# Anonymousijcai2024ttnet/scale_imagenet

Hardware: AMD Instinct MI355X
Metric: images/sec ImageNet 224x224, TT-small, MI355X; top-1 exact-match (higher is better)
Workload: dtype u16/u32/u64 packed bits (gate path); f32 as prescaled fp16x2 split operands on the 16-bit MFMA (stem, lin1, lin2); 1 GPU; TT_general_imagenet_v2_small forward, batch=256 224x224 per GPU, bit-packed HIP LUT kernels (BASELINE.json configs[1]); batch_per_gpu=256, global_batch=256, batches_in_flight=2, input=float32 NCHW, normalised (the reference's contract), parallelism=batch shard x1

## Files before the change

scale_imagenet_amd/csrc/head.hip:

```cpp

#include <algorithm>
#include <cmath>
#include <type_traits>

#include "ttnet_common.h"

namespace ttnet {

namespace {

typedef float f32x16 __attribute__((ext_vector_type(16)));

typedef _Float16 f16x8 __attribute__((ext_vector_type(8)));
constexpr int NP = SPLIT_PLANES;

#ifndef TT_LIN1_SKIP
#define TT_LIN1_SKIP 0
#endif
constexpr int kLin1Skip = TT_LIN1_SKIP;

#ifndef TT_LIN1_BM
#define TT_LIN1_BM 128
#endif
#ifndef TT_LIN1_WGS
#define TT_LIN1_WGS 256
#endif
constexpr int G_BM = TT_LIN1_BM, G_BN = 128;
constexpr int G_MT = G_BM / 32, G_NT = G_BN / 32;
constexpr int G_KS = 1;
constexpr int G_CHUNK = 1024;
constexpr int G_STAGE = (G_MT + G_NT) * G_KS * NP * G_CHUNK;
#ifndef TT_LIN1_STAGES
#define TT_LIN1_STAGES 4
#endif
constexpr int G_STAGES = TT_LIN1_STAGES;
#ifndef TT_LIN1_WAVES
#define TT_LIN1_WAVES (TT_LIN1_BM / 32)
#endif
constexpr int G_WAVES = TT_LIN1_WAVES;
constexpr int G_WN = G_WAVES / G_MT, NPW = G_NT / G_WN;
static_assert(G_WAVES % G_MT == 0 && G_NT % G_WN == 0, "waves tile the workgroup's output");
constexpr int G_CHUNKS = (G_MT + G_NT) * G_KS * NP;
#ifndef TT_LIN1_LOADERS
#define TT_LIN1_LOADERS 0
#endif
constexpr int G_LOADERS = TT_LIN1_LOADERS;
constexpr int G_THREADS = 64 * (G_WAVES + G_LOADERS);
constexpr int G_LW = G_LOADERS ? G_LOADERS : G_WAVES;
constexpr int G_LOADS = (G_CHUNKS + G_LW - 1) / G_LW;
constexpr int G_LDS = G_STAGES * G_STAGE + G_CHUNK;

#ifdef TT_LIN1_STAMP
__device__ unsigned long long g_lin1_stamps[512][2];
#endif
template <int AUX_A, int AUX_B>
__global__ __launch_bounds__(G_THREADS) void gemm_f16x2_kernel(const uint8_t *__restrict__ Af, const uint8_t *__restrict__ Bf,
                                                         float *__restrict__ part, int M, int N, int KS, int ks_per,
                                                         int n_tiles, int m_tiles, int splits) {
  extern __shared__ __align__(16) uint8_t lds[];
  const int lane = threadIdx.x & 63, wave = __builtin_amdgcn_readfirstlane(threadIdx.x >> 6);
  const bool loader = G_LOADERS ? wave >= G_WAVES : true, consumer = wave < G_WAVES;
  const int lw = G_LOADERS ? (loader ? wave - G_WAVES : 0) : wave;
  int ntile, mtile, slice;
  {
    const int b = blockIdx.x, groups = m_tiles * splits;
    const int lanes8 = groups < 8 ? groups : 8;
    const int round = b / (lanes8 * n_tiles), rem = b % (lanes8 * n_tiles);
    int grp = round * lanes8 + rem % lanes8;
    ntile = rem / lanes8;
    if (round == groups / lanes8) {
      const int left = groups - round * lanes8;
      grp = round * lanes8 + rem % left;
      ntile = rem / left;
    }
    mtile = grp / splits;
    slice = grp % splits;
  }
  const int mt0 = mtile * G_MT, nt0 = ntile * G_NT;
  const int ks_beg = slice * ks_per, iters = ks_per / G_KS;

  const uint8_t *chunk_src[G_LOADS];
  int chunk_lds[G_LOADS];
#pragma unroll
  for (int jj = 0; jj < G_LOADS; ++jj) {
    const int c = lw + G_LW * jj;
    const bool real = c < G_CHUNKS;
    const bool isA = c < G_MT * G_KS * NP;
    const int cc = real ? (isA ? c : c - G_MT * G_KS * NP) : 0;
    const int pl = cc % NP, kk = (cc / NP) % G_KS, tl = cc / (NP * G_KS);
    chunk_src[jj] = (isA || !real ? Af : Bf) +
                    ((((size_t)((isA || !real ? mt0 : nt0) + tl) * KS + ks_beg + kk) * NP + pl) * 64 + lane) * 16;
    chunk_lds[jj] = real ? c * G_CHUNK : -1;
  }
  auto issue = [&](int it, int buf) {
    static_for<0, G_LOADS>([&](auto jc) {
      constexpr int jj = decltype(jc)::value;
      constexpr bool allA = G_LW * jj + G_LW - 1 < G_MT * G_KS * NP, allB = G_LW * jj >= G_MT * G_KS * NP;
      if constexpr (kLin1Skip & 3) {
        const bool isA = lw + G_LW * jj < G_MT * G_KS * NP;
        if (((kLin1Skip & 1) && isA) || ((kLin1Skip & 2) && !isA)) return;
      }
      const auto src = (const __attribute__((address_space(1))) void *)(chunk_src[jj] + (size_t)it * (G_KS * NP * G_CHUNK));
      const auto dst = (__attribute__((address_space(3))) void *)(lds + (chunk_lds[jj] >= 0 ? buf * G_STAGE + chunk_lds[jj] : G_STAGES * G_STAGE));
      if constexpr (allA) __builtin_amdgcn_global_load_lds(src, dst, 16, 0, AUX_A);
      else if constexpr (allB) __builtin_amdgcn_global_load_lds(src, dst, 16, 0, AUX_B);
      else __builtin_amdgcn_global_load_lds(src, dst, 16, 0, 0);
    });
  };

  constexpr int MPW = 1;
  const int wm = wave % G_MT, wn = wave / G_MT;
  f32x16 acc[MPW][NPW];
#pragma unroll
  for (int i = 0; i < MPW; ++i)
#pragma unroll
    for (int j = 0; j < NPW; ++j)
#pragma unroll
      for (int r = 0; r < 16; ++r) acc[i][j][r] = 0.f;

  static_assert(G_KS == 1 && MPW == 1 && NPW == 4, "the fragment pipeline below is written for one k-step per stage and four N-tiles per wave");
  auto wait_landed = [&](int younger) {
    if (younger >= 5) asm volatile("s_waitcnt vmcnt(%0)" ::"n"(5 * G_LOADS) : "memory");
    else if (younger == 4) asm volatile("s_waitcnt vmcnt(%0)" ::"n"(4 * G_LOADS) : "memory");
    else if (younger == 3) asm volatile("s_waitcnt vmcnt(%0)" ::"n"(3 * G_LOADS) : "memory");
    else if (younger == 2) asm volatile("s_waitcnt vmcnt(%0)" ::"n"(2 * G_LOADS) : "memory");
    else if (younger == 1) asm volatile("s_waitcnt vmcnt(%0)" ::"n"(G_LOADS) : "memory");
    else asm volatile("s_waitcnt vmcnt(0)" ::: "memory");
  };
  static_assert(G_STAGES >= 4 && G_STAGES <= 8 && 5 * G_LOADS < 64, "G_STAGES - 1 stages issued ahead; the barrier of k-step it frees slot (it - 1) % G_STAGES");
#ifdef TT_LIN1_STAMP
  const unsigned long long st_c = __builtin_amdgcn_s_memtime(), st_r = __builtin_amdgcn_s_memrealtime();
#endif
  if (loader) {
    for (int p = 0; p < G_STAGES - 1 && p < iters; ++p) issue(p, p);
    wait_landed(min(G_STAGES - 2, iters - 1));
  }
  __builtin_amdgcn_s_barrier();
  typedef uint32_t u32x4 __attribute__((ext_vector_type(4)));
  u32x4 af[2][NP], bq[NPW][NP];
#define TT_DSRD(dst, addr, off) asm volatile("ds_read_b128 %0, %1 offset:%2" : "=&v"(dst) : "v"(addr), "n"(off))
  const uint32_t lds0 = (uint32_t)(uintptr_t)(__attribute__((address_space(3))) void *)lds + (uint32_t)lane * 16u;
  const uint32_t offA = (uint32_t)(wm * NP) * G_CHUNK, offB = (uint32_t)(G_MT * NP + wn * NPW * NP) * G_CHUNK;
  auto tile = [&](int j, const u32x4 (&a_cur)[NP]) {
    if constexpr (kLin1Skip & 4) {
      acc[0][j][0] += __uint_as_float(a_cur[0][0] ^ bq[j][0][0] ^ bq[j][1][0] ^ a_cur[1][0]);
    } else {
      const f16x8 a0 = __builtin_bit_cast(f16x8, a_cur[0]), a1 = __builtin_bit_cast(f16x8, a_cur[1]);
      const f16x8 b0 = __builtin_bit_cast(f16x8, bq[j][0]), b1 = __builtin_bit_cast(f16x8, bq[j][1]);
      acc[0][j] = __builtin_amdgcn_mfma_f32_32x32x16_f16(a1, b0, acc[0][j], 0, 0, 0);
      acc[0][j] = __builtin_amdgcn_mfma_f32_32x32x16_f16(a0, b1, acc[0][j], 0, 0, 0);
      acc[0][j] = __builtin_amdgcn_mfma_f32_32x32x16_f16(a0, b0, acc[0][j], 0, 0, 0);
    }
    __builtin_amdgcn_sched_barrier(0);
  };
  auto kstep = [&](auto par_c, int it) {
    constexpr int P = decltype(par_c)::value;
    u32x4 (&a_cur)[NP] = af[P];
    u32x4 (&a_nxt)[NP] = af[1 - P];
    const uint32_t sb = lds0 + (uint32_t)(it % G_STAGES) * G_STAGE + offB;
    const uint32_t sn = lds0 + (uint32_t)((it + 1) % G_STAGES) * G_STAGE;
    const uint32_t snb = sn + offB, sna = sn + offA;
    TT_DSRD(bq[2][0], sb, 4 * G_CHUNK);
    TT_DSRD(bq[2][1], sb, 5 * G_CHUNK);
    asm volatile("s_waitcnt lgkmcnt(4)" : "+v"(bq[0][0]), "+v"(bq[0][1]), "+v"(a_cur[0]), "+v"(a_cur[1]));
    tile(0, a_cur);
    TT_DSRD(bq[3][0], sb, 6 * G_CHUNK);
    TT_DSRD(bq[3][1], sb, 7 * G_CHUNK);
    asm volatile("s_waitcnt lgkmcnt(4)" : "+v"(bq[1][0]), "+v"(bq[1][1]));
    tile(1, a_cur);
    TT_DSRD(bq[0][0], snb, 0);
    TT_DSRD(bq[0][1], snb, G_CHUNK);
    TT_DSRD(a_nxt[0], sna, 0);
    TT_DSRD(a_nxt[1], sna, G_CHUNK);
    asm volatile("s_waitcnt lgkmcnt(6)" : "+v"(bq[2][0]), "+v"(bq[2][1]));
    tile(2, a_cur);
    TT_DSRD(bq[1][0], snb, 2 * G_CHUNK);
    TT_DSRD(bq[1][1], snb, 3 * G_CHUNK);
    asm volatile("s_waitcnt lgkmcnt(6)" : "+v"(bq[3][0]), "+v"(bq[3][1]));
    tile(3, a_cur);
  };
  if (consumer) {
    const uint32_t s0 = lds0;
    TT_DSRD(bq[0][0], s0 + offB, 0);
    TT_DSRD(bq[0][1], s0 + offB, G_CHUNK);
    TT_DSRD(af[0][0], s0 + offA, 0);
    TT_DSRD(af[0][1], s0 + offA, G_CHUNK);
    TT_DSRD(bq[1][0], s0 + offB, 2 * G_CHUNK);
    TT_DSRD(bq[1][1], s0 + offB, 3 * G_CHUNK);
  }
  auto step = [&](auto par_c, int it) {
    if (loader) wait_landed(max(0, min(it + G_STAGES - 2, iters - 1) - (it + 1)));
    __builtin_amdgcn_s_barrier();
    if (loader && it + G_STAGES - 1 < iters) issue(it + G_STAGES - 1, (it + G_STAGES - 1) % G_STAGES);
    if (consumer) kstep(par_c, it);
  };
#pragma unroll 1
  for (int it = 0; it < iters; it += 2) {
    step(std::integral_constant<int, 0>{}, it);
    if (it + 1 < iters) step(std::integral_constant<int, 1>{}, it + 1);
  }
  if (consumer)
    asm volatile("s_waitcnt lgkmcnt(0)" : "+v"(bq[0][0]), "+v"(bq[0][1]), "+v"(bq[1][0]), "+v"(bq[1][1]), "+v"(af[0][0]), "+v"(af[0][1]),
                 "+v"(af[1][0]), "+v"(af[1][1]));
#undef TT_DSRD
#ifdef TT_LIN1_STAMP
  if (threadIdx.x == 0 && blockIdx.x < 512) {
    g_lin1_stamps[blockIdx.x][0] = __builtin_amdgcn_s_memtime() - st_c;
    g_lin1_stamps[blockIdx.x][1] = 10ull * (__builtin_amdgcn_s_memrealtime() - st_r);
  }
#endif
  if (!consumer) return;
  float4 *dst = (float4 *)part + (size_t)slice * (m_tiles * G_MT) * (n_tiles * G_NT) * 256;
#pragma unroll
  for (int i = 0; i < MPW; ++i)
#pragma unroll
    for (int j = 0; j < NPW; ++j) {
      float4 *tile = dst + ((size_t)(mt0 + wm + i) * (n_tiles * G_NT) + nt0 + wn * NPW + j) * 256 + lane;
#pragma unroll
      for (int g = 0; g < 4; ++g) {
        if ((kLin1Skip & 8) && g) continue;
        tile[g * 64] = make_float4(acc[i][j][4 * g], acc[i][j][4 * g + 1], acc[i][j][4 * g + 2], acc[i][j][4 * g + 3]);
      }
    }
}

__global__ void split_to_frag_kernel(const float *__restrict__ src, uint16_t *__restrict__ dst, int R, int K, int tiles,
                                     float prescale, int ld, int kvalid) {
  const size_t i = (size_t)blockIdx.x * blockDim.x + threadIdx.x;
  const int KS = K / 16;
  if (i >= (size_t)tiles * KS * 64 * 8) return;
  const int j = i % 8, ln = (i / 8) % 64;
  const size_t tk = i / 512;
  const int ks = tk % KS, tl = tk / KS;
  const int row = tl * 32 + (ln & 31), k = ks * 16 + 8 * (ln >> 5) + j;
  const float v = row < R && k < kvalid ? src[(size_t)row * ld + k] * prescale : 0.f;
  uint16_t h1, h2;
  split_f16x2(v, h1, h2);
  const size_t base = ((size_t)tl * KS + ks) * NP;
  dst[((base + 0) * 64 + ln) * 8 + j] = h1;
  dst[((base + 1) * 64 + ln) * 8 + j] = h2;
}

__global__ void frag_to_ref_kernel(const uint16_t *__restrict__ af, float *__restrict__ out, int n, int G, int PP) {
  const size_t t = (size_t)blockIdx.x * blockDim.x + threadIdx.x;
  const size_t per = (size_t)G * PP * 16;
  if (t >= (size_t)n * per) return;
  const int kk = t % 16, pp = (t / 16) % PP, g = (t / (16 * (size_t)PP)) % G;
  const int img = t / per;
  out[(size_t)img * per + ((size_t)(16 * g + kk)) * PP + pp] = load_feature(af, img, G * PP, g * PP + pp, kk);
}

__global__ void head_mid_kernel(const float4 *__restrict__ part, int splits, const float *__restrict__ scale,
                                const float *__restrict__ shift, uint16_t *__restrict__ mid_frag, int M, int N,
                                int polynomial, uint32_t *range_flag, int mt32, int nt32) {
  const size_t i = (size_t)blockIdx.x * blockDim.x + threadIdx.x;
  const size_t per_slice = (size_t)mt32 * nt32 * 256;
// ... 53 lines not shown
        const f16x8 b0 = __builtin_bit_cast(f16x8, fb[sl][0]), b1 = __builtin_bit_cast(f16x8, fb[sl][1]);
        acc = __builtin_amdgcn_mfma_f32_32x32x16_f16(a1, b0, acc, 0, 0, 0);
        acc = __builtin_amdgcn_mfma_f32_32x32x16_f16(a0, b1, acc, 0, 0, 0);
        acc = __builtin_amdgcn_mfma_f32_32x32x16_f16(a0, b0, acc, 0, 0, 0);
        if (i0 + sl + L2_STAGES < nk) load(i0 + sl + L2_STAGES, fa[sl], fb[sl]);
      }
    });
  }
#pragma unroll
  for (int r = 0; r < 16; ++r) red[(wave * 16 + r) * 64 + lane] = acc[r];
  __syncthreads();
  for (int e = threadIdx.x; e < 16 * 64; e += 64 * L2_WAVES) {
    double sum = 0.0;
#pragma unroll
    for (int w = 0; w < L2_WAVES; ++w) sum += (double)red[w * (16 * 64) + e];
    const int ln = e & 63, r = e >> 6;
    const int row = mt * 32 + (r & 3) + 8 * (r >> 2) + 4 * (ln >> 5);
    const int col = nt * 32 + (ln & 31);
    if (row < M && col < N) out[(size_t)row * N + col] = (float)(sum * (double)inv + (double)bias[col]);
  }
}

__global__ void permute_lin1_kernel(const float *__restrict__ w1, float *__restrict__ w1p, int O, int G, int PP) {
  const size_t i = (size_t)blockIdx.x * blockDim.x + threadIdx.x;
  const size_t K = (size_t)G * PP * 16;
  if (i >= (size_t)O * K) return;
  const size_t o = i / K, f = i % K;
  const int k = f % 16, pp = (f / 16) % PP, g = f / (16 * (size_t)PP);
  w1p[i] = w1[o * K + ((size_t)(16 * g + k)) * PP + pp];
}

}

int gemm_f16x2_splits(int M, int N, int KS) {
  const int tiles = ((M + G_BM - 1) / G_BM) * ((N + G_BN - 1) / G_BN);
  const int want = std::max(TT_LIN1_WGS / std::max(1, tiles), 8);
  for (int s = std::min(std::min(want, KS / 8), 128); s > 1; --s)
    if (KS % s == 0) return s;
  return 1;
}

size_t gemm_f16x2_part_elems(int M, int N, int KS) {
  const size_t mt = (M + G_BM - 1) / G_BM, nt = (N + G_BN - 1) / G_BN;
  return (size_t)gemm_f16x2_splits(M, N, KS) * mt * G_BM * nt * G_BN;
}

int launch_gemm_f16x2(const void *Af, const void *Bf, float *part, int M, int N, int K, int splits, hipStream_t s) {
  const int KS = K / 16;
  if (K % 16 || KS % splits || (KS / splits) % G_KS) {
    set_error("gemm_f16x2: K=%d not divisible into %d slices of %d k-steps", K, splits, G_KS);
    return TTNET_E_UNSUPPORTED;
  }
  static const int nt = getenv("TTNET_LIN1_NT") ? atoi(getenv("TTNET_LIN1_NT")) : 0;
  const int n_tiles = (N + G_BN - 1) / G_BN, m_tiles = (M + G_BM - 1) / G_BM;
  auto launch = [&](auto kernel) -> int {
    TT_TRY(ensure_dynamic_lds((const void *)kernel, G_LDS));
    hipLaunchKernelGGL(kernel, dim3(n_tiles * m_tiles * splits), dim3(G_THREADS), G_LDS, s, (const uint8_t *)Af, (const uint8_t *)Bf, part, M, N,
                       KS, KS / splits, n_tiles, m_tiles, splits);
    return TTNET_OK;
  };
  if (nt == 11) TT_TRY(launch(gemm_f16x2_kernel<2, 2>));
  else if (nt == 1) TT_TRY(launch(gemm_f16x2_kernel<0, 2>));
  else if (nt == 10) TT_TRY(launch(gemm_f16x2_kernel<2, 0>));
  else TT_TRY(launch(gemm_f16x2_kernel<0, 0>));
  TT_HIP(hipGetLastError());
  return TTNET_OK;
}

size_t frag_elems(int rows, int K) { return (size_t)((rows + 31) / 32) * (K / 16) * NP * 64 * 8; }

float weight_prescale(const float *w, size_t n) {
  float amax = 0.f;
  for (size_t i = 0; i < n; ++i) amax = fmaxf(amax, fabsf(w[i]));
  if (!(amax > 0.f) || !std::isfinite(amax)) return 1.0f;
  int e;
  frexpf(amax, &e);
  int k = 14 - e;
  k = k > 60 ? 60 : (k < -60 ? -60 : k);
  return ldexpf(1.0f, k);
}

int launch_split_to_frag(const float *src, void *dst, int R, int K, int rows_padded, float prescale, hipStream_t s, int ld,
                         int kvalid) {
  if (K % 16) {
    set_error("split_to_frag: K=%d is not a multiple of 16", K);
    return TTNET_E_UNSUPPORTED;
  }
  const int tiles = (rows_padded + 31) / 32;
  const size_t t = (size_t)tiles * (K / 16) * 64 * 8;
  hipLaunchKernelGGL(split_to_frag_kernel, dim3((unsigned)((t + 255) / 256)), dim3(256), 0, s, src, (uint16_t *)dst, R, K, tiles,
                     prescale, ld > 0 ? ld : K, kvalid > 0 ? kvalid : K);
  TT_HIP(hipGetLastError());
  return TTNET_OK;
}

int launch_frag_to_reference_order(const void *af, float *out, int n, int G, int PP, hipStream_t s) {
  const size_t t = (size_t)n * G * PP * 16;
  hipLaunchKernelGGL(frag_to_ref_kernel, dim3((unsigned)((t + 255) / 256)), dim3(256), 0, s, (const uint16_t *)af, out, n, G, PP);
  TT_HIP(hipGetLastError());
  return TTNET_OK;
}

int launch_head_mid(const float *part, int splits, const float *scale, const float *shift, void *mid_frag, int M, int N,
                    int polynomial, uint32_t *range_flag, hipStream_t s) {
  const int mt32 = (M + G_BM - 1) / G_BM * G_MT, nt32 = (N + G_BN - 1) / G_BN * G_NT;
  const size_t t = (size_t)mt32 * nt32 * 256;
  hipLaunchKernelGGL(head_mid_kernel, dim3((unsigned)((t + 255) / 256)), dim3(256), 0, s, (const float4 *)part, splits, scale, shift,
                     (uint16_t *)mid_frag, M, N, polynomial, range_flag, mt32, nt32);
  TT_HIP(hipGetLastError());
  return TTNET_OK;
}

int launch_lin2_f16x2(const void *mid_frag, const void *w2f, const float *bias, float inv, float *out, int M, int N, int K,
                      hipStream_t s) {
  const int KS = (K + 15) / 16;
  hipLaunchKernelGGL(lin2_f16x2_kernel, dim3((N + 31) / 32, (M + 31) / 32), dim3(64 * L2_WAVES), 0, s,
                     (const uint4 *)mid_frag, (const uint4 *)w2f, bias, inv, out, M, N, KS);
  TT_HIP(hipGetLastError());
  return TTNET_OK;
}

int launch_permute_lin1(const float *w1, float *w1p, int O, int G, int PP, hipStream_t s) {
  const size_t t = (size_t)O * G * PP * 16;
  hipLaunchKernelGGL(permute_lin1_kernel, dim3((unsigned)((t + 255) / 256)), dim3(256), 0, s, w1, w1p, O, G, PP);
  TT_HIP(hipGetLastError());
  return TTNET_OK;
}

}
```

scale_imagenet_amd/csrc/plan.hip:

```cpp

#include <dlfcn.h>
#include <math.h>
#include <stdarg.h>
#include <stdint.h>
#include <stdio.h>
#include <stdlib.h>
#include <string.h>

#include <algorithm>
#include <array>
#include <map>
#include <memory>

#include <mutex>
#include <unordered_map>

#include "ttnet_common.h"

namespace ttnet {

static thread_local char g_err[1024] = "";

void set_error(const char *fmt, ...) {
  va_list ap;
// ... 411 lines not shown
        for (int b = 0; b < 4; ++b) TT_TRY(dev_alloc(pl, &bw.o[b], 8, true, ws));
        if (mh.last) TT_TRY(dev_alloc(pl, &bw.idx, (size_t)nb * (mh.C / 8) * mh.Ho * mh.Wo, true, ws));
        continue;
      }
      TT_TRY(dev_alloc(pl, &L.x_rp[i], (size_t)nb * mh.C * mh.H, true, ws));
      TT_TRY(dev_alloc(pl, &L.x_cp[i], path == GatePath::Full ? 8 : (size_t)nb * mh.H * mh.W * (mh.C / 16), true, ws));
      if (path == GatePath::Full) TT_TRY(dev_alloc(pl, &bw.c3_tmp, (size_t)nb * mh.C * mh.H, true, ws));
      for (int b = 0; b < 4; ++b) {
        const size_t words16 = (size_t)nb * mh.Ho * mh.Wo * (mh.C / 16), rows64 = (size_t)nb * mh.C * mh.Ho;
        TT_TRY(dev_alloc(pl, &bw.o[b], (path == GatePath::XSmall || path == GatePath::Full) ? rows64 * 4 : words16, true, ws));
      }
    }
    if (path == GatePath::Full) {
      const MultiHead &lb = pl->blocks.back();
      TT_TRY(dev_alloc(pl, &L.last_float, (size_t)nb * lb.cf.g.out_planes * lb.Ho * lb.Wo, true, ws));
      size_t cap = 0;
      for (const MultiHead &mh : pl->blocks) {
        cap = std::max(cap, (size_t)mh.c3.g.groups * mh.H * mh.W);
        if (!mh.last) cap = std::max(cap, (size_t)mh.cf.g.groups * mh.Ho * mh.Wo);
      }
      pl->full_fix_cap = cap * (size_t)nb;
      TT_TRY(dev_alloc(pl, &L.full_fix, 64 + pl->full_fix_cap, true, ws));
      if (!pl->full_gel) {
        TT_TRY(dev_alloc(pl, &pl->full_gel, full_gelu_tables_elems(), false, ws));
        TT_TRY(launch_full_gelu_tables(pl->full_gel, nullptr));
        TT_HIP(hipDeviceSynchronize());
      }
    }
  }
  const int nb_pad = (nb + 255) / 256 * 256;
  TT_TRY(dev_alloc(pl, &L.feat, frag_elems(nb_pad, pl->fcsize), true, ws));
  TT_TRY(dev_alloc(pl, &L.mid_frag, frag_elems((nb + 63) / 64 * 64, kpad), true, ws));
  size_t pe = 0;
  for (int n = 1; n <= nb; n = n < 256 ? 256 : n + 256) pe = std::max(pe, gemm_f16x2_part_elems(std::min(n, nb), pl->inter, pl->fcsize / 16));
  pe = std::max(pe, gemm_f16x2_part_elems(nb, pl->inter, pl->fcsize / 16));
  pl->part_elems = pe;
  TT_TRY(dev_alloc(pl, &L.part, pe, false, ws));
  return TTNET_OK;
}

int allocate(ttnet_plan *pl) {
  size_t *tb = &pl->table_bytes;
  TT_HIP(hipHostMalloc((void **)&pl->range_host, sizeof(uint32_t), hipHostMallocMapped));
  *pl->range_host = 0u;
  TT_HIP(hipHostGetDevicePointer((void **)&pl->range_dev, pl->range_host, 0));
  const int kpad = (pl->inter + 15) / 16 * 16;
  for (auto &kv : pl->tensors) TT_TRY(dev_alloc(pl, (uint8_t **)&kv.second.dev, kv.second.bytes, true));
  const bool valexnet = pl->path == GatePath::VAlexnet;
  if (valexnet) {
    TT_TRY(dev_alloc(pl, &pl->va_scale, 64, false));
    TT_TRY(dev_alloc(pl, &pl->va_shift, 64, false));
  } else {
    TT_TRY(dev_alloc(pl, &pl->stem_wt, stem_split_weights_elems(), false));
    TT_TRY(dev_alloc(pl, &pl->stem_init, 64, false));
    TT_TRY(dev_alloc(pl, &pl->norm_tab, stem_u8_table_elems(), true));
    TT_TRY(dev_alloc(pl, &pl->stem_wt_u8, stem_split_weights_elems(), true));
    TT_TRY(dev_alloc(pl, &pl->stem_init_u8, 64, true));
    TT_TRY(dev_alloc(pl, &pl->w1p, (size_t)pl->inter * pl->fcsize, false));
  }
  for (auto &mh : pl->blocks) {
    for (BlockTT *b : {&mh.c1, &mh.c2, &mh.c3, &mh.cf}) {
      if (valexnet && b == &mh.cf) continue;
      const BlockGeom &g = b->g;
      if (pl->path != GatePath::Full) {
        TT_TRY(dev_alloc(pl, (uint8_t **)&b->table, g.table_bytes(), true, tb));
        TT_TRY(dev_alloc(pl, &b->perm_dev, b->perm.size(), false));
        TT_HIP(hipMemcpy(b->perm_dev, b->perm.data(), b->perm.size(), hipMemcpyHostToDevice));
// ... 240 lines not shown
    a.groups = b.g.groups; a.cin = b.g.cin_g(); a.mid = b.g.mid_g(); a.cout = b.g.cout_g(); a.Cout = b.g.out_planes;
    a.Csrc = mh.C; a.interleaved = 1;
    for (int k = 0; k < 4; ++k) a.src[k] = o64[k];
    a.w1 = wts(b, ".conv1.weight"); a.w2 = wts(b, ".conv2.weight");
    a.s1 = b.s1; a.t1 = b.t1; a.s2 = b.s2; a.t2 = b.t2;
    a.gel = pl->full_gel ? pl->full_gel + full_gelu_tables_elems() / 2 : nullptr;
    a.fix_count = L.full_fix; a.fix_list = L.full_fix ? L.full_fix + 64 : nullptr; a.range_flag = pl->range_dev;
    if (mh.last) {
      a.out_rp = nullptr; a.out_float = L.last_float;
      TT_TIMED(pl, "full.convf_last", s, launch_full_pw(a, s));
      TT_TIMED(pl, "full.pool", s, launch_full_pool_split(L.last_float, L.feat, n, b.g.out_planes, mh.Ho, mh.Wo, pl->range_dev, s));
    } else {
      a.out_rp = L.x_rp[i + 1]; a.out_float = nullptr;
      static const char *const kCf[4] = {"full.convf.f4", "full.convf.f5", "full.convf.f6", "full.convf.f7"};
      TT_TIMED(pl, kCf[std::min<size_t>(i, 3)], s, launch_full_pw(a, s));
    }
  }
  return TTNET_OK;
}

int prepare_lin2(ttnet_plan *pl, const std::string &key, hipStream_t s) {
  std::vector<float> w2;
  TT_TRY(fetch(pl->tensors[key], w2));
  const float ws2 = weight_prescale(w2.data(), w2.size());
  pl->lin2_inv = 1.0f / (ws2 * ACT_PRESCALE);
  const int kpad = (pl->inter + 15) / 16 * 16;
  return launch_split_to_frag((const float *)pl->tensors[key].dev, pl->w2f, pl->n_classes, kpad, (pl->n_classes + 63) / 64 * 64, ws2, s,
                              pl->inter, pl->inter);
}

int run_head(ttnet_plan *pl, const ttnet_plan::Lane &L, int n, float *logits, hipStream_t s) {
  const int polynomial = pl->path == GatePath::VAlexnet ? 0 : 1;
  const int s1 = gemm_f16x2_splits(n, pl->inter, pl->fcsize / 16);
  TT_TIMED(pl, "head.lin1", s, launch_gemm_f16x2(L.feat, pl->w1f, L.part, n, pl->inter, pl->fcsize, s1, s));
  TT_TIMED(pl, polynomial ? "head.bn_poly" : "head.bn", s,
           launch_head_mid(L.part, s1, pl->bn_scale, pl->bn_shift, L.mid_frag, n, pl->inter, polynomial, pl->range_dev, s));
  TT_TIMED(pl, "head.lin2", s,
           launch_lin2_f16x2(L.mid_frag, pl->w2f, (const float *)pl->tensors[pl->head + ".lin2.bias"].dev, pl->lin2_inv, logits, n,
                             pl->n_classes, pl->inter, s));
  return TTNET_OK;
}

int run_from_blocks(ttnet_plan *pl, ttnet_plan::Lane &L, int n, float *logits, hipStream_t s) {
  for (size_t i = 0; i < pl->blocks.size(); ++i) {
    switch (pl->path) {
      case GatePath::TwoLaunch: TT_TRY(run_two_launch_block(pl, L, i, n, s)); break;
      case GatePath::Fused: TT_TRY(run_fused_block(pl, L, i, n, s)); break;
      case GatePath::XSmall: TT_TRY(run_xs_block(pl, L, i, n, s)); break;
      case GatePath::Full: TT_TRY(run_full_block(pl, L, i, n, s)); break;
      case GatePath::VAlexnet: TT_TRY(run_va_block(pl, L, n, s)); break;
    }
  }
  TT_TRY(run_head(pl, L, n, logits, s));
  L.last_n = n;
  return TTNET_OK;
}

int check_range(ttnet_plan *pl) {
  if (pl->range_host && *(volatile uint32_t *)pl->range_host) {
    set_error("an earlier forward on this plan met an activation outside the range of the fp16 x 2 operand split "
              "(|input| or |feature| >= 4094, or NaN): its logits are invalid; ttnet_plan_query(\"range_overflow\") "
              "reads and clears the flag");
    return TTNET_E_RANGE;
  }
  return TTNET_OK;
}
// ... 816 lines not shown
```

scale_imagenet_amd/csrc/ttnet_common.h:

```cpp
#pragma once

#include <hip/hip_runtime.h>
#include <stdint.h>
#include <algorithm>
#include <string>
#include <type_traits>
#include <vector>

#include "../../include/ttnet.h"

namespace ttnet {

void set_error(const char *fmt, ...);

#define TT_HIP(call)                                                                       \
  do {                                                                                     \
    hipError_t e__ = (call);                                                               \
    if (e__ != hipSuccess) {                                                               \
      ::ttnet::set_error("%s failed: %s (%s:%d)", #call, hipGetErrorString(e__), __FILE__, \
                         __LINE__);                                                        \
      return TTNET_E_HIP;                                                                  \
    }                                                                                      \
  } while (0)

// ... 208 lines not shown
  uint32_t fix_cap;
  float tau_scale;
  const float *gel;
};
struct FullPwArgs {
  int n, H, W;
  int groups, cin, mid, cout, Cout;
  int Csrc;
  int interleaved;
  const uint64_t *src[4];
  const float *w1, *w2;
  const double *s1, *t1, *s2, *t2;
  uint64_t *out_rp;
  float *out_float;
  uint32_t *fix_list, *fix_count, *range_flag;
  float tau_scale;
  const float *gel;
};
int launch_full_dw(const FullDwArgs &a, hipStream_t s);
int launch_full_pw(const FullPwArgs &a, hipStream_t s);
size_t full_gelu_tables_elems();
int launch_full_gelu_tables(float *dst, hipStream_t s);
int launch_rp_majority(const uint64_t *x, uint64_t *out, int n, int C, int H, int W, int Ho, int pad_t, int pad_l,
                       hipStream_t s);
int launch_full_pool_split(const float *x, void *feat_frag, int n, int C, int H, int W, uint32_t *range_flag, hipStream_t s);
int launch_va_stem(const float *x, const float *w, const float *bias, const float *scale, const float *shift,
                   uint64_t *rp, int n, hipStream_t s);
int launch_va_block(const uint64_t *x_rp, const void *t1, const void *t2, const void *t3, uint64_t *y, int n, hipStream_t s);
int launch_va_feat(const uint64_t *y, void *feat_frag, int n, hipStream_t s);
int launch_va_frag_to_flat(const void *af, float *out, int n, hipStream_t s);
int launch_cp_to_rp(const uint16_t *cp, uint64_t *rp, int n, int C, int H, int W, hipStream_t s);
int launch_rp_to_cp(const uint64_t *rp, uint16_t *cp, int n, int C, int H, int W, hipStream_t s);
int launch_frag_to_reference_order(const void *af, float *out, int n, int G, int PP, hipStream_t s);
int gemm_f16x2_splits(int M, int N, int KS);
size_t gemm_f16x2_part_elems(int M, int N, int KS);
int launch_gemm_f16x2(const void *Af, const void *Bf, float *part, int M, int N, int K, int splits, hipStream_t s);
size_t frag_elems(int rows, int K);
int launch_split_to_frag(const float *src, void *dst, int R, int K, int rows_padded, float prescale, hipStream_t s, int ld = 0,
                         int kvalid = 0);

int launch_head_mid(const float *part, int splits, const float *scale, const float *shift, void *mid_frag, int M, int N,
                    int polynomial, uint32_t *range_flag, hipStream_t s);
int launch_lin2_f16x2(const void *mid_frag, const void *w2f, const float *bias, float inv, float *out, int M, int N, int K,
                      hipStream_t s);
int launch_permute_lin1(const float *w1, float *w1p, int O, int G, int PP, hipStream_t s);

}
```

Baseline: 1.985 million images/s.

## Restructure lin1 GEMM so each wave owns an N-tile with B held in registers

Reworks the split-K f16x2 GEMM for the head's first linear layer. Each of four waves now owns one 32-wide N-tile and loads its B fragments straight into a ring of registers with global_load_dwordx4. Only A goes through LDS, and waves sweep all M-tiles while rotating four A register sets. This cuts LDS traffic and footprint for B and drops the loader-wave variants and cache-policy template knobs. An optional env-selected 256-row tile is added, and the workspace sizing loop and a bounds check are adjusted. The cost is higher register pressure and a different load/wait schedule.

```diff
diff --git a/scale_imagenet_amd/csrc/head.hip b/scale_imagenet_amd/csrc/head.hip
--- a/scale_imagenet_amd/csrc/head.hip
+++ b/scale_imagenet_amd/csrc/head.hip
@@ -19,48 +19,32 @@
 #endif
 constexpr int kLin1Skip = TT_LIN1_SKIP;
 
-#ifndef TT_LIN1_BM
-#define TT_LIN1_BM 128
-#endif
+constexpr int G_BN = 128, G_NT = G_BN / 32;
+constexpr int G_WAVES = 4, G_THREADS = 64 * G_WAVES;
+static_assert(G_WAVES == G_NT, "wave w owns N-tile w");
+constexpr int G_CHUNK = 1024;
+#ifndef TT_LIN1_STAGES
+#define TT_LIN1_STAGES 4
+#endif
+constexpr int G_STAGES = TT_LIN1_STAGES;
 #ifndef TT_LIN1_WGS
 #define TT_LIN1_WGS 256
 #endif
-constexpr int G_BM = TT_LIN1_BM, G_BN = 128;
-constexpr int G_MT = G_BM / 32, G_NT = G_BN / 32;
-constexpr int G_KS = 1;
-constexpr int G_CHUNK = 1024;
-constexpr int G_STAGE = (G_MT + G_NT) * G_KS * NP * G_CHUNK;
-#ifndef TT_LIN1_STAGES
-#define TT_LIN1_STAGES 4
-#endif
-constexpr int G_STAGES = TT_LIN1_STAGES;
-#ifndef TT_LIN1_WAVES
-#define TT_LIN1_WAVES (TT_LIN1_BM / 32)
-#endif
-constexpr int G_WAVES = TT_LIN1_WAVES;
-constexpr int G_WN = G_WAVES / G_MT, NPW = G_NT / G_WN;
-static_assert(G_WAVES % G_MT == 0 && G_NT % G_WN == 0, "waves tile the workgroup's output");
-constexpr int G_CHUNKS = (G_MT + G_NT) * G_KS * NP;
-#ifndef TT_LIN1_LOADERS
-#define TT_LIN1_LOADERS 0
-#endif
-constexpr int G_LOADERS = TT_LIN1_LOADERS;
-constexpr int G_THREADS = 64 * (G_WAVES + G_LOADERS);
-constexpr int G_LW = G_LOADERS ? G_LOADERS : G_WAVES;
-constexpr int G_LOADS = (G_CHUNKS + G_LW - 1) / G_LW;
-constexpr int G_LDS = G_STAGES * G_STAGE + G_CHUNK;
 
 #ifdef TT_LIN1_STAMP
 __device__ unsigned long long g_lin1_stamps[512][2];
 #endif
-template <int AUX_A, int AUX_B>
+template <int MT>
 __global__ __launch_bounds__(G_THREADS) void gemm_f16x2_kernel(const uint8_t *__restrict__ Af, const uint8_t *__restrict__ Bf,
                                                          float *__restrict__ part, int M, int N, int KS, int ks_per,
                                                          int n_tiles, int m_tiles, int splits) {
+  constexpr int STAGE = MT * NP * G_CHUNK;
+  constexpr int LA = (kLin1Skip & 1) ? 0 : MT * NP / G_WAVES, LB = (kLin1Skip & 2) ? 0 : NP;
+  constexpr int LOADS = LA + LB;
+  static_assert(MT % 4 == 0 && (MT * NP) % G_WAVES == 0, "the fragment pipeline rotates four A register sets per k-step");
+  static_assert(G_STAGES >= 4 && G_STAGES <= 8 && G_STAGES * STAGE <= 65536 && (G_STAGES - 2) * LOADS < 64, "ring and wait counts");
   extern __shared__ __align__(16) uint8_t lds[];
   const int lane = threadIdx.x & 63, wave = __builtin_amdgcn_readfirstlane(threadIdx.x >> 6);
-  const bool loader = G_LOADERS ? wave >= G_WAVES : true, consumer = wave < G_WAVES;
-  const int lw = G_LOADERS ? (loader ? wave - G_WAVES : 0) : wave;
   int ntile, mtile, slice;
   {
     const int b = blockIdx.x, groups = m_tiles * splits;
@@ -76,132 +60,120 @@
     mtile = grp / splits;
     slice = grp % splits;
   }
-  const int mt0 = mtile * G_MT, nt0 = ntile * G_NT;
-  const int ks_beg = slice * ks_per, iters = ks_per / G_KS;
-
-  const uint8_t *chunk_src[G_LOADS];
-  int chunk_lds[G_LOADS];
-#pragma unroll
-  for (int jj = 0; jj < G_LOADS; ++jj) {
-    const int c = lw + G_LW * jj;
-    const bool real = c < G_CHUNKS;
-    const bool isA = c < G_MT * G_KS * NP;
-    const int cc = real ? (isA ? c : c - G_MT * G_KS * NP) : 0;
-    const int pl = cc % NP, kk = (cc / NP) % G_KS, tl = cc / (NP * G_KS);
-    chunk_src[jj] = (isA || !real ? Af : Bf) +
-                    ((((size_t)((isA || !real ? mt0 : nt0) + tl) * KS + ks_beg + kk) * NP + pl) * 64 + lane) * 16;
-    chunk_lds[jj] = real ? c * G_CHUNK : -1;
-  }
-  auto issue = [&](int it, int buf) {
-    static_for<0, G_LOADS>([&](auto jc) {
+  const int mt0 = mtile * MT, nt0 = ntile * G_NT;
+  const int ks_beg = slice * ks_per, iters = ks_per;
+
+  const uint8_t *a_src[LA ? LA : 1];
+#pragma unroll
+  for (int jj = 0; jj < LA; ++jj) {
+    const int c = wave + G_WAVES * jj;
+    a_src[jj] = Af + ((((size_t)(mt0 + c / NP) * KS + ks_beg) * NP + c % NP) * 64 + lane) * 16;
+  }
+  const uint8_t *b_src = Bf + (((size_t)(nt0 + wave) * KS + ks_beg) * NP * 64 + lane) * 16;
+  typedef uint32_t u32x4 __attribute__((ext_vector_type(4)));
+  u32x4 bq[G_STAGES][NP];
+  u32x4 af[4][NP];
+#pragma unroll
+  for (int q = 0; q < G_STAGES; ++q)
+#pragma unroll
+    for (int pl = 0; pl < NP; ++pl) bq[q][pl] = u32x4{0u, 0u, 0u, 0u};
+  auto issue = [&](int it, auto slot_c) {
+    constexpr int slot = decltype(slot_c)::value;
+    u32x4 (&b_set)[NP] = bq[slot];
+    static_for<0, LA>([&](auto jc) {
       constexpr int jj = decltype(jc)::value;
-      constexpr bool allA = G_LW * jj + G_LW - 1 < G_MT * G_KS * NP, allB = G_LW * jj >= G_MT * G_KS * NP;
-      if constexpr (kLin1Skip & 3) {
-        const bool isA = lw + G_LW * jj < G_MT * G_KS * NP;
-        if (((kLin1Skip & 1) && isA) || ((kLin1Skip & 2) && !isA)) return;
+      const auto src = (const __attribute__((address_space(1))) void *)(a_src[jj] + (size_t)it * (NP * G_CHUNK));
+      const auto dst = (__attribute__((address_space(3))) void *)(lds + slot * STAGE + (wave + G_WAVES * jj) * G_CHUNK);
+      __builtin_amdgcn_global_load_lds(src, dst, 16, 0, 0);
+    });
+    static_for<0, LB>([&](auto pc) {
+      constexpr int pl = decltype(pc)::value;
+      const uint8_t *src = b_src + (size_t)it * (NP * G_CHUNK) + pl * G_CHUNK;
+      u32x4 &dst = b_set[pl];
+      asm volatile("global_load_dwordx4 %0, %1, off" : "+v"(dst) : "v"(src) : "memory");
+    });
+  };
+
+  f32x16 acc[MT];
+#pragma unroll
+  for (int i = 0; i < MT; ++i)
+#pragma unroll
+    for (int r = 0; r < 16; ++r) acc[i][r] = 0.f;
+
+  auto wait_landed = [&](int younger) {
+    bool done = false;
+    static_for<0, G_STAGES - 2>([&](auto kc) {
+      constexpr int k = G_STAGES - 2 - decltype(kc)::value;
+      if (!done && younger >= k) {
+        asm volatile("s_waitcnt vmcnt(%0)" ::"n"(k * LOADS) : "memory");
+        done = true;
       }
-      const auto src = (const __attribute__((address_space(1))) void *)(chunk_src[jj] + (size_t)it * (G_KS * NP * G_CHUNK));
-      const auto dst = (__attribute__((address_space(3))) void *)(lds + (chunk_lds[jj] >= 0 ? buf * G_STAGE + chunk_lds[jj] : G_STAGES * G_STAGE));
-      if constexpr (allA) __builtin_amdgcn_global_load_lds(src, dst, 16, 0, AUX_A);
-      else if constexpr (allB) __builtin_amdgcn_global_load_lds(src, dst, 16, 0, AUX_B);
-      else __builtin_amdgcn_global_load_lds(src, dst, 16, 0, 0);
-    });
-  };
-
-  constexpr int MPW = 1;
-  const int wm = wave % G_MT, wn = wave / G_MT;
-  f32x16 acc[MPW][NPW];
-#pragma unroll
-  for (int i = 0; i < MPW; ++i)
-#pragma unroll
-    for (int j = 0; j < NPW; ++j)
-#pragma unroll
-      for (int r = 0; r < 16; ++r) acc[i][j][r] = 0.f;
-
-  static_assert(G_KS == 1 && MPW == 1 && NPW == 4, "the fragment pipeline below is written for one k-step per stage and four N-tiles per wave");
-  auto wait_landed = [&](int younger) {
-    if (younger >= 5) asm volatile("s_waitcnt vmcnt(%0)" ::"n"(5 * G_LOADS) : "memory");
-    else if (younger == 4) asm volatile("s_waitcnt vmcnt(%0)" ::"n"(4 * G_LOADS) : "memory");
-    else if (younger == 3) asm volatile("s_waitcnt vmcnt(%0)" ::"n"(3 * G_LOADS) : "memory");
-    else if (younger == 2) asm volatile("s_waitcnt vmcnt(%0)" ::"n"(2 * G_LOADS) : "memory");
-    else if (younger == 1) asm volatile("s_waitcnt vmcnt(%0)" ::"n"(G_LOADS) : "memory");
-    else asm volatile("s_waitcnt vmcnt(0)" ::: "memory");
-  };
-  static_assert(G_STAGES >= 4 && G_STAGES <= 8 && 5 * G_LOADS < 64, "G_STAGES - 1 stages issued ahead; the barrier of k-step it frees slot (it - 1) % G_STAGES");
+    });
+    if (!done) asm volatile("s_waitcnt vmcnt(0)" ::: "memory");
+  };
+  auto landed = [&](auto slot_c) {
+    u32x4 (&b_set)[NP] = bq[decltype(slot_c)::value];
+    asm volatile("" : "+v"(b_set[0]), "+v"(b_set[1]));
+  };
 #ifdef TT_LIN1_STAMP
   const unsigned long long st_c = __builtin_amdgcn_s_memtime(), st_r = __builtin_amdgcn_s_memrealtime();
 #endif
-  if (loader) {
-    for (int p = 0; p < G_STAGES - 1 && p < iters; ++p) issue(p, p);
-    wait_landed(min(G_STAGES - 2, iters - 1));
-  }
+  static_for<0, G_STAGES - 1>([&](auto pc) {
+    if (decltype(pc)::value < iters) issue(decltype(pc)::value, pc);
+  });
+  wait_landed(min(G_STAGES - 2, iters - 1));
+  landed(std::integral_constant<int, 0>{});
   __builtin_amdgcn_s_barrier();
-  typedef uint32_t u32x4 __attribute__((ext_vector_type(4)));
-  u32x4 af[2][NP], bq[NPW][NP];
 #define TT_DSRD(dst, addr, off) asm volatile("ds_read_b128 %0, %1 offset:%2" : "=&v"(dst) : "v"(addr), "n"(off))
   const uint32_t lds0 = (uint32_t)(uintptr_t)(__attribute__((address_space(3))) void *)lds + (uint32_t)lane * 16u;
-  const uint32_t offA = (uint32_t)(wm * NP) * G_CHUNK, offB = (uint32_t)(G_MT * NP + wn * NPW * NP) * G_CHUNK;
-  auto tile = [&](int j, const u32x4 (&a_cur)[NP]) {
+  auto tile = [&](auto ic, const u32x4 (&b_cur)[NP]) {
+    constexpr int i = decltype(ic)::value;
     if constexpr (kLin1Skip & 4) {
-      acc[0][j][0] += __uint_as_float(a_cur[0][0] ^ bq[j][0][0] ^ bq[j][1][0] ^ a_cur[1][0]);
+      acc[i][0] += __uint_as_float(af[i % 4][0][0] ^ b_cur[0][0] ^ b_cur[1][0] ^ af[i % 4][1][0]);
     } else {
-      const f16x8 a0 = __builtin_bit_cast(f16x8, a_cur[0]), a1 = __builtin_bit_cast(f16x8, a_cur[1]);
-      const f16x8 b0 = __builtin_bit_cast(f16x8, bq[j][0]), b1 = __builtin_bit_cast(f16x8, bq[j][1]);
-      acc[0][j] = __builtin_amdgcn_mfma_f32_32x32x16_f16(a1, b0, acc[0][j], 0, 0, 0);
-      acc[0][j] = __builtin_amdgcn_mfma_f32_32x32x16_f16(a0, b1, acc[0][j], 0, 0, 0);
-      acc[0][j] = __builtin_amdgcn_mfma_f32_32x32x16_f16(a0, b0, acc[0][j], 0, 0, 0);
+      const f16x8 a0 = __builtin_bit_cast(f16x8, af[i % 4][0]), a1 = __builtin_bit_cast(f16x8, af[i % 4][1]);
+      const f16x8 b0 = __builtin_bit_cast(f16x8, b_cur[0]), b1 = __builtin_bit_cast(f16x8, b_cur[1]);
+      acc[i] = __builtin_amdgcn_mfma_f32_32x32x16_f16(a1, b0, acc[i], 0, 0, 0);
+      acc[i] = __builtin_amdgcn_mfma_f32_32x32x16_f16(a0, b1, acc[i], 0, 0, 0);
+      acc[i] = __builtin_amdgcn_mfma_f32_32x32x16_f16(a0, b0, acc[i], 0, 0, 0);
     }
     __builtin_amdgcn_sched_barrier(0);
   };
-  auto kstep = [&](auto par_c, int it) {
-    constexpr int P = decltype(par_c)::value;
-    u32x4 (&a_cur)[NP] = af[P];
-    u32x4 (&a_nxt)[NP] = af[1 - P];
-    const uint32_t sb = lds0 + (uint32_t)(it % G_STAGES) * G_STAGE + offB;
-    const uint32_t sn = lds0 + (uint32_t)((it + 1) % G_STAGES) * G_STAGE;
-    const uint32_t snb = sn + offB, sna = sn + offA;
-    TT_DSRD(bq[2][0], sb, 4 * G_CHUNK);
-    TT_DSRD(bq[2][1], sb, 5 * G_CHUNK);
-    asm volatile("s_waitcnt lgkmcnt(4)" : "+v"(bq[0][0]), "+v"(bq[0][1]), "+v"(a_cur[0]), "+v"(a_cur[1]));
-    tile(0, a_cur);
-    TT_DSRD(bq[3][0], sb, 6 * G_CHUNK);
-    TT_DSRD(bq[3][1], sb, 7 * G_CHUNK);
-    asm volatile("s_waitcnt lgkmcnt(4)" : "+v"(bq[1][0]), "+v"(bq[1][1]));
-    tile(1, a_cur);
-    TT_DSRD(bq[0][0], snb, 0);
-    TT_DSRD(bq[0][1], snb, G_CHUNK);
-    TT_DSRD(a_nxt[0], sna, 0);
-    TT_DSRD(a_nxt[1], sna, G_CHUNK);
-    asm volatile("s_waitcnt lgkmcnt(6)" : "+v"(bq[2][0]), "+v"(bq[2][1]));
-    tile(2, a_cur);
-    TT_DSRD(bq[1][0], snb, 2 * G_CHUNK);
-    TT_DSRD(bq[1][1], snb, 3 * G_CHUNK);
-    asm volatile("s_waitcnt lgkmcnt(6)" : "+v"(bq[3][0]), "+v"(bq[3][1]));
-    tile(3, a_cur);
-  };
-  if (consumer) {
-    const uint32_t s0 = lds0;
-    TT_DSRD(bq[0][0], s0 + offB, 0);
-    TT_DSRD(bq[0][1], s0 + offB, G_CHUNK);
-    TT_DSRD(af[0][0], s0 + offA, 0);
-    TT_DSRD(af[0][1], s0 + offA, G_CHUNK);
-    TT_DSRD(bq[1][0], s0 + offB, 2 * G_CHUNK);
-    TT_DSRD(bq[1][1], s0 + offB, 3 * G_CHUNK);
-  }
-  auto step = [&](auto par_c, int it) {
-    if (loader) wait_landed(max(0, min(it + G_STAGES - 2, iters - 1) - (it + 1)));
+  auto kstep = [&](auto slot_c) {
+    constexpr int slot = decltype(slot_c)::value;
+    const uint32_t sa = lds0 + (uint32_t)slot * STAGE, sn = lds0 + (uint32_t)((slot + 1) % G_STAGES) * STAGE;
+    static_for<0, MT>([&](auto ic) {
+      constexpr int i = decltype(ic)::value, r = i + 2;
+      if constexpr (r < MT) {
+        TT_DSRD(af[r % 4][0], sa, r * NP * G_CHUNK);
+        TT_DSRD(af[r % 4][1], sa, r * NP * G_CHUNK + G_CHUNK);
+      } else {
+        TT_DSRD(af[r % 4][0], sn, (r - MT) * NP * G_CHUNK);
+        TT_DSRD(af[r % 4][1], sn, (r - MT) * NP * G_CHUNK + G_CHUNK);
+      }
+      asm volatile("s_waitcnt lgkmcnt(4)" : "+v"(af[i % 4][0]), "+v"(af[i % 4][1]));
+      tile(ic, bq[slot]);
+    });
+  };
+  TT_DSRD(af[0][0], lds0, 0);
+  TT_DSRD(af[0][1], lds0, G_CHUNK);
+  TT_DSRD(af[1][0], lds0, NP * G_CHUNK);
+  TT_DSRD(af[1][1], lds0, NP * G_CHUNK + G_CHUNK);
+  auto step = [&](auto slot_c, int it) {
+    constexpr int slot = decltype(slot_c)::value;
+    wait_landed(max(0, min(it + G_STAGES - 2, iters - 1) - (it + 1)));
+    landed(std::integral_constant<int, (slot + 1) % G_STAGES>{});
     __builtin_amdgcn_s_barrier();
-    if (loader && it + G_STAGES - 1 < iters) issue(it + G_STAGES - 1, (it + G_STAGES - 1) % G_STAGES);
-    if (consumer) kstep(par_c, it);
+    if (it + G_STAGES - 1 < iters) issue(it + G_STAGES - 1, std::integral_constant<int, (slot + G_STAGES - 1) % G_STAGES>{});
+    kstep(slot_c);
   };
 #pragma unroll 1
-  for (int it = 0; it < iters; it += 2) {
-    step(std::integral_constant<int, 0>{}, it);
-    if (it + 1 < iters) step(std::integral_constant<int, 1>{}, it + 1);
-  }
-  if (consumer)
-    asm volatile("s_waitcnt lgkmcnt(0)" : "+v"(bq[0][0]), "+v"(bq[0][1]), "+v"(bq[1][0]), "+v"(bq[1][1]), "+v"(af[0][0]), "+v"(af[0][1]),
-                 "+v"(af[1][0]), "+v"(af[1][1]));
+  for (int it = 0; it < iters; it += G_STAGES)
+    static_for<0, G_STAGES>([&](auto sc) {
+      if (it + decltype(sc)::value < iters) step(sc, it + decltype(sc)::value);
+    });
+  asm volatile("s_waitcnt lgkmcnt(0)" : "+v"(af[0][0]), "+v"(af[0][1]), "+v"(af[1][0]), "+v"(af[1][1]), "+v"(af[2][0]), "+v"(af[2][1]),
+               "+v"(af[3][0]), "+v"(af[3][1]));
 #undef TT_DSRD
 #ifdef TT_LIN1_STAMP
   if (threadIdx.x == 0 && blockIdx.x < 512) {
@@ -209,19 +181,16 @@
     g_lin1_stamps[blockIdx.x][1] = 10ull * (__builtin_amdgcn_s_memrealtime() - st_r);
   }
 #endif
-  if (!consumer) return;
-  float4 *dst = (float4 *)part + (size_t)slice * (m_tiles * G_MT) * (n_tiles * G_NT) * 256;
-#pragma unroll
-  for (int i = 0; i < MPW; ++i)
-#pragma unroll
-    for (int j = 0; j < NPW; ++j) {
-      float4 *tile = dst + ((size_t)(mt0 + wm + i) * (n_tiles * G_NT) + nt0 + wn * NPW + j) * 256 + lane;
-#pragma unroll
-      for (int g = 0; g < 4; ++g) {
-        if ((kLin1Skip & 8) && g) continue;
-        tile[g * 64] = make_float4(acc[i][j][4 * g], acc[i][j][4 * g + 1], acc[i][j][4 * g + 2], acc[i][j][4 * g + 3]);
-      }
+  float4 *dst = (float4 *)part + (size_t)slice * (m_tiles * MT) * (n_tiles * G_NT) * 256;
+#pragma unroll
+  for (int i = 0; i < MT; ++i) {
+    float4 *tile = dst + ((size_t)(mt0 + i) * (n_tiles * G_NT) + nt0 + wave) * 256 + lane;
+#pragma unroll
+    for (int g = 0; g < 4; ++g) {
+      if ((kLin1Skip & 8) && g) continue;
+      tile[g * 64] = make_float4(acc[i][4 * g], acc[i][4 * g + 1], acc[i][4 * g + 2], acc[i][4 * g + 3]);
     }
+  }
 }
 
 __global__ void split_to_frag_kernel(const float *__restrict__ src, uint16_t *__restrict__ dst, int R, int K, int tiles,
@@ -341,37 +310,51 @@
 
 }
 
+static int lin1_env(const char *name) {
+  const char *v = getenv(name);
+  return v ? atoi(v) : 0;
+}
+
+int gemm_f16x2_bm(int M) {
+  static const int forced = lin1_env("TTNET_LIN1_BM");
+  (void)M;
+  return forced == 256 ? 256 : 128;
+}
+
 int gemm_f16x2_splits(int M, int N, int KS) {
-  const int tiles = ((M + G_BM - 1) / G_BM) * ((N + G_BN - 1) / G_BN);
-  const int want = std::max(TT_LIN1_WGS / std::max(1, tiles), 8);
+  static const int forced = lin1_env("TTNET_LIN1_SPLITS");
+  const int bm = gemm_f16x2_bm(M);
+  const int tiles = ((M + bm - 1) / bm) * ((N + G_BN - 1) / G_BN);
+  int want = std::max(TT_LIN1_WGS / std::max(1, tiles), 8);
+  if (bm == 256) want = std::min(want, 16);
+  if (forced > 0) want = forced;
   for (int s = std::min(std::min(want, KS / 8), 128); s > 1; --s)
     if (KS % s == 0) return s;
   return 1;
 }
 
 size_t gemm_f16x2_part_elems(int M, int N, int KS) {
-  const size_t mt = (M + G_BM - 1) / G_BM, nt = (N + G_BN - 1) / G_BN;
-  return (size_t)gemm_f16x2_splits(M, N, KS) * mt * G_BM * nt * G_BN;
+  const size_t bm = gemm_f16x2_bm(M), mt = (M + bm - 1) / bm, nt = (N + G_BN - 1) / G_BN;
+  return (size_t)gemm_f16x2_splits(M, N, KS) * mt * bm * nt * G_BN;
 }
 
 int launch_gemm_f16x2(const void *Af, const void *Bf, float *part, int M, int N, int K, int splits, hipStream_t s) {
   const int KS = K / 16;
-  if (K % 16 || KS % splits || (KS / splits) % G_KS) {
-    set_error("gemm_f16x2: K=%d not divisible into %d slices of %d k-steps", K, splits, G_KS);
+  if (K % 16 || splits < 1 || KS % splits) {
+    set_error("gemm_f16x2: K=%d not divisible into %d slices of whole k-steps", K, splits);
     return TTNET_E_UNSUPPORTED;
   }
-  static const int nt = getenv("TTNET_LIN1_NT") ? atoi(getenv("TTNET_LIN1_NT")) : 0;
-  const int n_tiles = (N + G_BN - 1) / G_BN, m_tiles = (M + G_BM - 1) / G_BM;
-  auto launch = [&](auto kernel) -> int {
-    TT_TRY(ensure_dynamic_lds((const void *)kernel, G_LDS));
-    hipLaunchKernelGGL(kernel, dim3(n_tiles * m_tiles * splits), dim3(G_THREADS), G_LDS, s, (const uint8_t *)Af, (const uint8_t *)Bf, part, M, N,
+  const int bm = gemm_f16x2_bm(M);
+  const int n_tiles = (N + G_BN - 1) / G_BN, m_tiles = (M + bm - 1) / bm;
+  auto launch = [&](auto kernel, int mt) -> int {
+    const size_t lds_bytes = (size_t)G_STAGES * mt * NP * G_CHUNK;
+    TT_TRY(ensure_dynamic_lds((const void *)kernel, lds_bytes));
+    hipLaunchKernelGGL(kernel, dim3(n_tiles * m_tiles * splits), dim3(G_THREADS), lds_bytes, s, (const uint8_t *)Af, (const uint8_t *)Bf, part, M, N,
                        KS, KS / splits, n_tiles, m_tiles, splits);
     return TTNET_OK;
   };
-  if (nt == 11) TT_TRY(launch(gemm_f16x2_kernel<2, 2>));
-  else if (nt == 1) TT_TRY(launch(gemm_f16x2_kernel<0, 2>));
-  else if (nt == 10) TT_TRY(launch(gemm_f16x2_kernel<2, 0>));
-  else TT_TRY(launch(gemm_f16x2_kernel<0, 0>));
+  if (bm == 256) TT_TRY(launch(gemm_f16x2_kernel<8>, 8));
+  else TT_TRY(launch(gemm_f16x2_kernel<4>, 4));
   TT_HIP(hipGetLastError());
   return TTNET_OK;
 }
@@ -412,7 +395,8 @@
 
 int launch_head_mid(const float *part, int splits, const float *scale, const float *shift, void *mid_frag, int M, int N,
                     int polynomial, uint32_t *range_flag, hipStream_t s) {
-  const int mt32 = (M + G_BM - 1) / G_BM * G_MT, nt32 = (N + G_BN - 1) / G_BN * G_NT;
+  const int bm = gemm_f16x2_bm(M);
+  const int mt32 = (M + bm - 1) / bm * (bm / 32), nt32 = (N + G_BN - 1) / G_BN * G_NT;
   const size_t t = (size_t)mt32 * nt32 * 256;
   hipLaunchKernelGGL(head_mid_kernel, dim3((unsigned)((t + 255) / 256)), dim3(256), 0, s, (const float4 *)part, splits, scale, shift,
                      (uint16_t *)mid_frag, M, N, polynomial, range_flag, mt32, nt32);
diff --git a/scale_imagenet_amd/csrc/plan.hip b/scale_imagenet_amd/csrc/plan.hip
--- a/scale_imagenet_amd/csrc/plan.hip
+++ b/scale_imagenet_amd/csrc/plan.hip
@@ -467,7 +467,7 @@
   TT_TRY(dev_alloc(pl, &L.feat, frag_elems(nb_pad, pl->fcsize), true, ws));
   TT_TRY(dev_alloc(pl, &L.mid_frag, frag_elems((nb + 63) / 64 * 64, kpad), true, ws));
   size_t pe = 0;
-  for (int n = 1; n <= nb; n = n < 256 ? 256 : n + 256) pe = std::max(pe, gemm_f16x2_part_elems(std::min(n, nb), pl->inter, pl->fcsize / 16));
+  for (int n = 1; n <= nb; n += 128) pe = std::max(pe, gemm_f16x2_part_elems(n, pl->inter, pl->fcsize / 16));
   pe = std::max(pe, gemm_f16x2_part_elems(nb, pl->inter, pl->fcsize / 16));
   pl->part_elems = pe;
   TT_TRY(dev_alloc(pl, &L.part, pe, false, ws));
@@ -774,6 +774,11 @@
 int run_head(ttnet_plan *pl, const ttnet_plan::Lane &L, int n, float *logits, hipStream_t s) {
   const int polynomial = pl->path == GatePath::VAlexnet ? 0 : 1;
   const int s1 = gemm_f16x2_splits(n, pl->inter, pl->fcsize / 16);
+  if (gemm_f16x2_part_elems(n, pl->inter, pl->fcsize / 16) > pl->part_elems) {
+    set_error("head: the split-K slabs of a batch of %d need %zu floats, the workspace holds %zu", n,
+              gemm_f16x2_part_elems(n, pl->inter, pl->fcsize / 16), pl->part_elems);
+    return TTNET_E_STATE;
+  }
   TT_TIMED(pl, "head.lin1", s, launch_gemm_f16x2(L.feat, pl->w1f, L.part, n, pl->inter, pl->fcsize, s1, s));
   TT_TIMED(pl, polynomial ? "head.bn_poly" : "head.bn", s,
            launch_head_mid(L.part, s1, pl->bn_scale, pl->bn_shift, L.mid_frag, n, pl->inter, polynomial, pl->range_dev, s));
diff --git a/scale_imagenet_amd/csrc/ttnet_common.h b/scale_imagenet_amd/csrc/ttnet_common.h
--- a/scale_imagenet_amd/csrc/ttnet_common.h
+++ b/scale_imagenet_amd/csrc/ttnet_common.h
@@ -264,6 +264,7 @@
 int launch_cp_to_rp(const uint16_t *cp, uint64_t *rp, int n, int C, int H, int W, hipStream_t s);
 int launch_rp_to_cp(const uint64_t *rp, uint16_t *cp, int n, int C, int H, int W, hipStream_t s);
 int launch_frag_to_reference_order(const void *af, float *out, int n, int G, int PP, hipStream_t s);
+int gemm_f16x2_bm(int M);
 int gemm_f16x2_splits(int M, int N, int KS);
 size_t gemm_f16x2_part_elems(int M, int N, int KS);
 int launch_gemm_f16x2(const void *Af, const void *Bf, float *part, int M, int N, int K, int splits, hipStream_t s);
```

Result: no change. 1.970 million images/s (-0.7%).
